# sail-sg/finetune-fair-diffusion

Measured on AMD Instinct MI355X. Metric: training-images/sec (SD-v1.5 512^2, 20-step DPM-Solver++ unroll, fairness-finetune step), higher is better.
Workload: dtype f16

## Files before the change

finetune_fair_diffusion_amd/ops.py:

```python
import ctypes
import os
import math

import torch

from . import lib as _lib

ACT = dict(none=0, silu=1, quick_gelu=2, gelu=3, relu=4, hardswish=5, hardsigmoid=6, geglu=7)
CONV_NORMAL, CONV_STRIDE2, CONV_UP2, CONV_TRANS2 = 0, 1, 2, 3
F16, F32 = _lib.torch_working_dtype(), torch.float32


def _stream():
    return ctypes.c_void_p(torch.cuda.current_stream().cuda_stream)


def _p(t):
    if t is None:
        return None
    assert t.is_cuda, "fairdiff ops need device tensors (no CPU path)"
    return ctypes.c_void_p(t.data_ptr())


DELAY = None


def _call(name, *args):
    if DELAY is not None and DELAY[2].random() < DELAY[0]:
        torch.cuda._sleep(int(DELAY[2].random() * DELAY[1]))
    L = _lib.get()
    rc = getattr(L, name)(*args)
    if rc != 0:
        raise RuntimeError(f"{name} failed ({rc}): {L.fd_last_error().decode()}")


_gemm_ws = {}


def gemm_workspace():
    dev = torch.cuda.current_device()
    key = (dev, torch.cuda.current_stream().cuda_stream)
    t = _gemm_ws.get(key)
    if t is None:
        t = torch.empty(16 << 20, dtype=F32, device=torch.device("cuda", dev))
        _gemm_ws[key] = t
    return t


class OpTimer:

    def __init__(self):
        self.shapes = []
        self.records = []

    def summary(self):
        torch.cuda.synchronize()
        agg = {}
        for variant, flops, nbytes, a, b, split in self.records:
            ms = a.elapsed_time(b)
            e = agg.setdefault(variant, [0, 0.0, 0.0, 0.0, 0])
            e[0] += 1; e[1] += flops; e[2] += ms; e[3] += nbytes; e[4] += int(split)
        self.by_shape = {}
        for (variant, flops, nbytes, a, b, split), shp in zip(self.records, self.shapes):
            e = self.by_shape.setdefault((variant,) + shp, [0, 0.0, 0.0])
            e[0] += 1; e[1] += flops; e[2] += a.elapsed_time(b)
        return {k: dict(launches=v[0], flops=v[1], ms=v[2], bytes=v[3], splitk_launches=v[4]) for k, v in agg.items()}

    def shape_table(self):
        rows = [k + (v[0], v[2], 1e3 * v[2] / v[0], v[1] / (v[2] * 1e-3) / 1e12) for k, v in self.by_shape.items()]
        return sorted(rows, key=lambda r: -r[10])


TIMER = None


GN_STATS = os.environ.get("FD_NO_GN_STATS") is None

def _gemm_call(d, conv, out=None, gn_stats=False):
    ws = gemm_workspace()
    d.workspace, d.workspace_bytes = ws.data_ptr(), ws.numel() * 4
    if gn_stats and GN_STATS:
        rows = _lib.get().fd_gemm_stats_rows(ctypes.byref(d))
        if rows > 0:
            nph = 4 if (conv and d.conv_mode == CONV_UP2PI) else 1
            st = torch.empty((nph * ((d.M + rows - 1) // rows), d.N // 10, 2), dtype=F32, device=out.device)
            d.gn_stats = st.data_ptr()
            out.gn_stats = (st, rows)
    if TIMER is None:
        _call("fd_gemm", ctypes.byref(d), _stream())
        return
    buf = ctypes.create_string_buffer(128)
    split = _lib.get().fd_gemm_kernel_name(ctypes.byref(d), buf, 128)
    a, b = torch.cuda.Event(enable_timing=True), torch.cuda.Event(enable_timing=True)
    a.record()
    _call("fd_gemm", ctypes.byref(d), _stream())
    b.record()
    nph = 4 if (conv and d.conv_mode in (4, 6)) else 1
    flops = 2.0 * nph * d.M * d.N * (d.K + d.K2) * max(d.batch, 1)
    a_elems = (d.Bn * d.H * d.W * d.Cin) if conv else d.M * d.K
    nbytes = 2.0 * max(d.batch, 1) * (a_elems + d.M * d.K2 + nph * d.N * (d.K + d.K2) + nph * d.M * d.N)
    TIMER.records.append((buf.value.decode(), flops, nbytes, a, b, split > 1))
    TIMER.shapes.append((d.M, d.N, d.K, d.K2, d.conv_mode if conv else -1, int(d.act), int(bool(d.residual)), split))


def _chk(t, dtype=F16):
    assert t.dtype == dtype and t.is_contiguous(), (t.dtype, t.shape, t.stride())
    return t


def gemm(a, b, *, a2=None, b2=None, bias=None, rowbias=None, rows_per_batch=0, residual=None, act="none", alpha=1.0,
         out=None, out_dtype=F16, n=None, aux=None, gn_stats=False, ln=None, colscale=None):
    M, K = a.shape
    N = b.shape[0] if n is None else n
    assert b.shape[1] == K and a.stride(1) == 1 and b.stride(1) == 1
    if out is None:
        out = torch.empty((M, N // 2 if act == "geglu" else N), dtype=out_dtype, device=a.device)
    d = _lib.GemmDesc()
    d.A, d.lda, d.B, d.ldb = a.data_ptr(), a.stride(0), b.data_ptr(), b.stride(0)
    if a2 is not None:
        assert a2.shape[0] == M and a2.shape[1] == b2.shape[1] and a2.stride(1) == 1 and b2.stride(1) == 1
        d.A2, d.lda2, d.B2, d.ldb2, d.K2 = a2.data_ptr(), a2.stride(0), b2.data_ptr(), b2.stride(0), a2.shape[1]
    d.C, d.ldc = out.data_ptr(), out.stride(0)
    if bias is not None:
        d.bias = _chk(bias, F32).data_ptr()
    if rowbias is not None:
        d.rowbias, d.ld_rowbias, d.rows_per_batch = _chk(rowbias).data_ptr(), rowbias.stride(0), rows_per_batch
    if residual is not None:
        assert residual.dtype == F16 and residual.stride(1) == 1
        d.residual, d.ldr = residual.data_ptr(), residual.stride(0)
    if aux is not None:
        assert act == "geglu" and residual is None and aux.shape == (M, N) and aux.dtype == F16 and aux.is_contiguous()
        d.residual, d.ldr = aux.data_ptr(), N
    d.alpha, d.M, d.N, d.K = alpha, M, N, K
    d.act, d.out_dtype, d.batch = ACT[act], 1 if out.dtype == F32 else 0, 1
    if colscale is not None:
        d.colscale, d.colscale_cols = colscale
    if ln is None:
        _gemm_call(d, False, out, gn_stats)
        return out
    _gemm_call(d, False, out, False)
    y, st = layernorm(out, ln[0], ln[1], ln[2], save_stats=True)
    return out, y, st


def interleave_geglu(w, bias):
    F = w.shape[0] // 2
    wi = torch.stack([w[:F], w[F:]], dim=1).reshape(2 * F, w.shape[1]).contiguous()
    bi = torch.stack([bias[:F], bias[F:]], dim=1).reshape(2 * F).contiguous() if bias is not None else None
    return wi, bi


def bgemm(a, b, *, alpha=1.0, out=None):
    Z, M, K = a.shape
    N = b.shape[1]
    _chk(a), _chk(b)
    if out is None:
        out = torch.empty((Z, M, N), dtype=F16, device=a.device)
    d = _lib.GemmDesc()
    d.A, d.lda, d.B, d.ldb, d.C, d.ldc = a.data_ptr(), K, b.data_ptr(), K, out.data_ptr(), N
    d.alpha, d.M, d.N, d.K, d.batch = alpha, M, N, K, Z
    d.sA, d.sB, d.sC = M * K, N * K, M * N
    _gemm_call(d, False)
    return out


def gemm_batched_into(a, b, out_view, bias, residual, Z, rows):
    K, N = a.shape[1], b.shape[0]
    assert a.shape[0] == Z * rows and out_view.shape == (Z, rows, N) and out_view.stride(2) == 1 and a.is_contiguous()
    d = _lib.GemmDesc()
    d.A, d.lda, d.B, d.ldb = a.data_ptr(), K, b.data_ptr(), b.stride(0)
    d.C, d.ldc = out_view.data_ptr(), out_view.stride(1)
    if bias is not None:
        d.bias = _chk(bias, F32).data_ptr()
    if residual is not None:
        d.residual, d.ldr, d.sR = _chk(residual).data_ptr(), residual.stride(0), 0
    d.alpha, d.M, d.N, d.K, d.batch = 1.0, rows, N, K, Z
    d.sA, d.sB, d.sC = rows * K, 0, out_view.stride(0)
    _gemm_call(d, False)
    return out_view


def gemm_batched_from(a_view, b, Z, rows):
    K, N = a_view.shape[2], b.shape[0]
    assert a_view.shape[:2] == (Z, rows) and a_view.stride(2) == 1 and b.shape[1] == K
    out = torch.empty((Z * rows, N), dtype=F16, device=b.device)
    d = _lib.GemmDesc()
    d.A, d.lda, d.B, d.ldb = a_view.data_ptr(), a_view.stride(1), b.data_ptr(), b.stride(0)
    d.C, d.ldc = out.data_ptr(), N
    d.alpha, d.M, d.N, d.K, d.batch = 1.0, rows, N, K, Z
    d.sA, d.sB, d.sC = a_view.stride(0), 0, rows * N
    _gemm_call(d, False)
    return out


def conv3x3(x, w, B, H, W, *, mode=CONV_NORMAL, bias=None, rowbias=None, residual=None, act="none", out=None, gn_stats=False):
    Cin = x.shape[1]
    Cout = w.shape[0]
    assert w.shape[1] == 9 * Cin and x.shape[0] == B * H * W
    _chk(x), _chk(w)
    if mode == CONV_NORMAL:
        Ho, Wo = H, W
    elif mode == CONV_STRIDE2:
        Ho, Wo = (H + 1) // 2, (W + 1) // 2
    else:
        Ho, Wo = 2 * H, 2 * W
    M = B * Ho * Wo
    if out is None:
        out = torch.empty((M, Cout), dtype=F16, device=x.device)
    d = _lib.GemmDesc()
    d.A, d.lda, d.B, d.ldb, d.C, d.ldc = x.data_ptr(), Cin, w.data_ptr(), 9 * Cin, out.data_ptr(), out.stride(0)
    if bias is not None:
        d.bias = _chk(bias, F32).data_ptr()
    if rowbias is not None:
        d.rowbias, d.ld_rowbias, d.rows_per_batch = _chk(rowbias).data_ptr(), rowbias.stride(0), (M if rowbias.shape[0] == 1 else Ho * Wo)
    if residual is not None:
        d.residual, d.ldr = _chk(residual).data_ptr(), residual.stride(0)
    d.alpha, d.M, d.N, d.K, d.act, d.batch = 1.0, M, Cout, 9 * Cin, ACT[act], 1
    d.out_dtype = 1 if out.dtype == F32 else 0
    d.conv, d.conv_mode, d.Bn, d.H, d.W, d.Cin, d.Ho, d.Wo = 1, mode, B, H, W, Cin, Ho, Wo
    _gemm_call(d, True, out, gn_stats)
    return out, Ho, Wo


CONV_UP2P, CONV_UP2P_BWD, CONV_UP2PI = 4, 5, 6
_BIG_TILES = (256320, 128320, 128160, 256128, 256256, 512128)
_NO_UP2P = os.environ.get("FD_NO_UP2P") is not None


def _up2p_desc(x, w, out, B, H, W, Cin, Cout, bwd, bias=None):
    d = _lib.GemmDesc()
    if bwd:
        d.K, d.conv_mode, d.H, d.W = 16 * Cin, CONV_UP2P_BWD, 2 * H, 2 * W
    else:
        d.K, d.conv_mode, d.H, d.W = 4 * Cin, CONV_UP2PI, H, W
    d.A, d.lda, d.B, d.ldb, d.C, d.ldc = x.data_ptr(), Cin, w.data_ptr(), d.K, out.data_ptr(), Cout
    if bias is not None:
        d.bias = _chk(bias, F32).data_ptr()
    d.alpha, d.M, d.N, d.act, d.batch, d.out_dtype = 1.0, B * H * W, Cout, ACT["none"], 1, 0
    d.conv, d.Bn, d.Cin, d.Ho, d.Wo = 1, B, Cin, H, W
    ws = gemm_workspace()
    d.workspace, d.workspace_bytes = ws.data_ptr(), ws.numel() * 4
    return d


def conv_up2(x, conv, B, H, W):
    Cin, Cout = conv.cin, conv.cout
    if not _NO_UP2P and Cin % 64 == 0 and Cout % 8 == 0:
        out = torch.empty((4 * B * H * W, Cout), dtype=F16, device=x.device)
        d = _up2p_desc(_chk(x), conv.wk_up2p, out, B, H, W, Cin, Cout, False, conv.bias)
        if _lib.get().fd_gemm_tile(ctypes.byref(d)) in _BIG_TILES:
            _gemm_call(d, True, out, gn_stats=(H * W) % 32 == 0)
            if getattr(out, "gn_stats", None) is not None:
                out.gn_stats = out.gn_stats + ((H * W) // 32,)
            return out, 2 * H, 2 * W
    return conv3x3(x, conv.wk, B, H, W, mode=CONV_UP2, bias=conv.bias)


def conv_up2_bwd(dy, conv, B, H, W):
    Cin, Cout = conv.cin, conv.cout
    if not _NO_UP2P and Cout % 64 == 0 and Cin % 8 == 0:
        out = torch.empty((B * H * W, Cin), dtype=F16, device=dy.device)
        d = _up2p_desc(_chk(dy), conv.wd_up2p, out, B, H, W, Cout, Cin, True)
        if _lib.get().fd_gemm_tile(ctypes.byref(d)) % 1000000 in _BIG_TILES:
            _gemm_call(d, True)
            return out
    dxu, _, _ = conv3x3(dy, conv.wd, B, 2 * H, 2 * W)
    return downsum2x2(dxu, B, H, W, Cin)


def conv_small_cin(x, w, bias, B, H, W, Cin, Cout, k, stride=1, nchw=True, act="none"):
    pad = (k - 1) // 2
    Ho, Wo = (H + 2 * pad - k) // stride + 1, (W + 2 * pad - k) // stride + 1
    y = torch.empty((B * Ho * Wo, Cout), dtype=F16, device=x.device)
    assert x.is_contiguous() and x.dtype in (F16, F32)
    _call("fd_conv_small_cin", _p(x), int(x.dtype == F32), int(nchw), _p(_chk(w, F32)), _p(bias), _p(y), B, H, W, Cin, Cout, k, stride,
          ACT[act], _stream())
    return y, Ho, Wo


def conv_small_cin_bwd(dy, w, B, H, W, Cin, Cout, k, stride=1, scale=1.0):
    dx = torch.empty((B, Cin, H, W), dtype=F32, device=dy.device)
    _call("fd_conv_small_cin_bwd", _p(_chk(dy)), _p(_chk(w, F32)), _p(dx), B, H, W, Cin, Cout, k, stride, scale, _stream())
    return dx


def nhwc_to_nchw(x, B, HW, C, *, out_dtype=F32, scale=1.0, lo=-math.inf, hi=math.inf):
    y = torch.empty((B, C, HW), dtype=out_dtype, device=x.device)
    _call("fd_nhwc_to_nchw", _p(x), x.stride(0), _p(y), int(out_dtype == F32), B, HW, C, scale, lo, hi, _stream())
    return y


def clamp_bwd(pre, dimg, B, HW, C, lo=-1.0, hi=1.0):
    out = torch.empty_like(dimg)
    _call("fd_clamp_bwd", _p(pre), pre.stride(0), _p(_chk(dimg, F32)), _p(out), B, HW, C, lo, hi, _stream())
    return out
# ... 432 lines not shown
```

finetune_fair_diffusion_amd/unet.py:

```python
import math

import torch

from . import ops
from .layers import (F16, F32, Conv3x3, Linear, LoRAPair, Norm, ParamBank, ResnetBlock, lora_linear_bwd, lora_linear_fwd)
from .weights import UNetConfig, unet_attn_names, unet_lora_param_shapes, unet_param_shapes


BWD_SLOT = [None]


class _Out:
    def __init__(self, sample):
        self.sample = sample


class LoRAAttnProcessor:

    def __init__(self, hidden_size, cross_attention_dim=None, rank=4):
        self.hidden_size, self.cross_attention_dim, self.rank = hidden_size, cross_attention_dim, rank

    def to(self, *a, **k):
        return self


class AttnLoRA:

    def __init__(self, bank, name):
        self.q, self.k, self.v, self.out = (LoRAPair(bank, f"{name}.{p}_lora.down.weight", f"{name}.{p}_lora.up.weight")
                                            for p in ("to_q", "to_k", "to_v", "to_out"))
        dev = bank.flat.device
        rp = self.q.rp
        if self.q.K == self.k.K:
            C = self.q.N
            self.down_qkv16 = torch.zeros((3 * rp, C), dtype=F16, device=dev)
            self.down_qkvT16 = torch.zeros((C, 3 * rp), dtype=F16, device=dev)
            self.up_qkv16 = torch.zeros((3 * C, 3 * rp), dtype=F16, device=dev)
            self.upT_qkv16 = torch.zeros((3 * rp, 3 * C), dtype=F16, device=dev)
            for i, p in enumerate((self.q, self.k, self.v)):
                p.place(self.down_qkv16[i * rp:(i + 1) * rp], self.down_qkvT16[:, i * rp:(i + 1) * rp],
                        self.up_qkv16[i * C:(i + 1) * C, i * rp:(i + 1) * rp], self.upT_qkv16[i * rp:(i + 1) * rp, i * C:(i + 1) * C])
            self.down_kv16 = self.down_qkv16[rp:]
        else:
            self.down_kv16 = torch.zeros((2 * rp, self.k.K), dtype=F16, device=dev)
            self.q.place()
            self.k.place(down16=self.down_kv16[:rp])
            self.v.place(down16=self.down_kv16[rp:])
        self.out.place()

    def pairs(self):
        return (self.q, self.k, self.v, self.out)

    def refresh(self):
        from .layers import refresh_pairs
        refresh_pairs(self.pairs())


class TransformerBlock:

    def __init__(self, sd, p, dev, C, heads, groups, xdim):
        self.C, self.heads, self.d, self.groups, self.xdim = C, heads, C // heads, groups, xdim
        self.p = p
        self.norm = Norm(sd, p + "norm", dev)
        self.proj_in = Linear(sd, p + "proj_in", dev, conv1x1=True)
        self.proj_out = Linear(sd, p + "proj_out", dev, conv1x1=True)
        b = p + "transformer_blocks.0."
        self.ln1, self.ln2, self.ln3 = Norm(sd, b + "norm1", dev), Norm(sd, b + "norm2", dev), Norm(sd, b + "norm3", dev)
        self.q1, self.k1, self.v1, self.o1 = (Linear(sd, b + "attn1." + n, dev) for n in ("to_q", "to_k", "to_v", "to_out.0"))
        assert self.q1.bias is None and self.k1.bias is None and self.v1.bias is None
        self.wqkv = torch.cat([self.q1.w, self.k1.w, self.v1.w], 0).contiguous()
        self._wqkvT = None
        self.q2, self.k2, self.v2, self.o2 = (Linear(sd, b + "attn2." + n, dev) for n in ("to_q", "to_k", "to_v", "to_out.0"))
        ff1, self.ff2 = Linear(sd, b + "ff.net.0.proj", dev), Linear(sd, b + "ff.net.2", dev)
        self.ff1_wi, self.ff1_bi = ops.interleave_geglu(ff1.w, ff1.bias)
        self._ff1_wiT = None
        self.lora1 = self.lora2 = None
        self.name1, self.name2 = b + "attn1.processor", b + "attn2.processor"
        self.cross = None
        self.lean = False

    def prepare_cross(self, enc, Bk, L, record, static=False):
        lo = self.lora2
        te = ops.gemm(enc, lo.down_kv16) if lo is not None else None
        rp = lo.k.rp if lo is not None else 0
        old = None
        if lo is not None:
            K = ops.gemm(enc, self.k2.w, a2=te[:, :rp], b2=lo.k.up16)
            V = ops.gemm(enc, self.v2.w, a2=te[:, rp:], b2=lo.v.up16)
        elif static:
            old = self.cross if (self.cross is not None and self.cross.get("static") and self.cross["K"].shape == (Bk * L, self.C)) else None
            K = ops.gemm(enc, self.k2.w, out=old["K"] if old else None)
            V = ops.gemm(enc, self.v2.w, out=old["V"] if old else None)
            if old is None:
                self.static_generation = getattr(self, "static_generation", 0) + 1
        else:
            K, V = ops.gemm(enc, self.k2.w), ops.gemm(enc, self.v2.w)
        self.cross = dict(static=bool(static and lo is None), K=K, V=V, Bk=Bk, L=L, enc=enc, te=te)
        if ops.FUSED_CROSS and L <= ops.CROSS_LP and self.C in ops.CROSS_WIDTHS and self.heads == 8:
            self.cross["Vt80"] = ops.transpose_btc(V, Bk, L, self.C, ops.CROSS_LP, out=old.get("Vt80") if (static and old) else None)
        if record:
            self.cross["dK"] = torch.zeros((Bk * L, self.C), dtype=F32, device=enc.device)
            self.cross["dV"] = torch.zeros((Bk * L, self.C), dtype=F32, device=enc.device)

    def finish_cross_backward(self, gscale, need_denc):
        c, lo = self.cross, self.lora2
        if c.get("slots") is not None:
            c["dK"] += c["slots"][:, 0].sum(dim=0)
            c["dV"] += c["slots"][:, 1].sum(dim=0)
            c["slots"] = None
        dK, dV = ops.to_f16(c["dK"]), ops.to_f16(c["dV"])
        rp = lo.k.rp if lo is not None else 0
        te = c["te"]
        denc = lora_linear_bwd(dK, c["enc"], te[:, :rp] if te is not None else None, self.k2, lo.k if lo else None, gscale, need_dx=need_denc)
        denc = lora_linear_bwd(dV, c["enc"], te[:, rp:] if te is not None else None, self.v2, lo.v if lo else None, gscale, residual=denc,
                               need_dx=need_denc)
        return denc

    def forward(self, x, B, H, W, ctx=None, pair=False):
        HW, C, h, d = H * W, self.C, self.heads, self.d
        rec = ctx is not None
        g, st = ops.groupnorm(x, None, B, HW, self.groups, 1e-6, self.norm.gamma, self.norm.beta, False)
        h0, n1, ln1 = ops.gemm(g, self.proj_in.w, bias=self.proj_in.bias, ln=(self.ln1.gamma, self.ln1.beta, 1e-5))
        l1 = self.lora1
        qs = ops.q_prescale(d)
        csq = (qs, C) if qs is not None else None
        if l1 is not None:
            t1 = ops.gemm(n1, l1.down_qkv16)
            qkv = ops.gemm(n1, self.wqkv, a2=t1, b2=l1.up_qkv16, colscale=csq)
        else:
            t1 = None
            qkv = ops.gemm(n1, self.wqkv, colscale=csq)
        q, k, v = qkv[:, :C], qkv[:, C:2 * C], qkv[:, 2 * C:]
        o, lse = ops.attn_fwd(q, k, v, B, h, HW, HW, d, 1, need_lse=True, prescaled=qs is not None)
        l2 = self.lora2
        cr = self.cross
        if (not pair and cr.get("Vt80") is not None and self.q2.bias is None and self.o2.bias is not None and (ops.FUSED_CROSS_TRAIN or (not rec and l2 is None))
                and ops.cross_block_ok(B * HW, C, h, cr["L"], HW, l2.q.rp if l2 is not None else 0)):
            h1, to1 = lora_linear_fwd(o, self.o1, l1.out if l1 else None, residual=h0)
            qs2 = ops.q_prescale(d)
            h2, n3, ln3, r = ops.cross_attn_block(h1, (self.ln2.gamma, self.ln2.beta, 1e-5), self.q2.w, cr["K"], cr["Vt80"], cr["L"], self.o2.w, self.o2.bias,
                                                  (self.ln3.gamma, self.ln3.beta, 1e-5), h, HW, B // cr["Bk"], lora_q=l2.q if l2 else None,
                                                  lora_o=l2.out if l2 else None, record=rec, q_prescaled=qs2 is not None)
            lean = rec and self.lean
            proj = torch.empty((n3.shape[0], self.ff1_wi.shape[0]), dtype=F16, device=n3.device) if rec and not lean else None
            gg = ops.gemm(n3, self.ff1_wi, bias=self.ff1_bi, act="geglu", aux=proj)
            h3 = ops.gemm(gg, self.ff2.w, bias=self.ff2.bias, residual=h2)
            out = ops.gemm(h3, self.proj_out.w, bias=self.proj_out.bias, residual=x, gn_stats=True)
            if rec:
                ctx.append(dict(x=x, st=st, h0=h0, ln1=ln1, n1=None if lean else n1, t1=t1, qkv=qkv, o=o, lse=lse, to1=to1, h1=h1, ln2=r["ln2"], n2=None if lean else r["n2"], tq2=r["tq2"], q2=r["q2"],
                                o2=r["o2"], lse2=r["lse2"], to2=r["to2"], h2=h2, ln3=ln3, proj=proj, pair=False, qs=qs is not None, qs2=qs2 is not None))
            return out
        (h1, n2, ln2), to1 = lora_linear_fwd(o, self.o1, l1.out if l1 else None, residual=h0, ln=(self.ln2.gamma, self.ln2.beta, 1e-5))
        qs2 = ops.q_prescale(d)
        q2, tq2 = lora_linear_fwd(n2, self.q2, l2.q if l2 else None, colscale=(qs2, C) if qs2 is not None else None)
        B2 = 2 * B if pair else B
        q2f, h1f, xf = (torch.cat([q2, q2]), torch.cat([h1, h1]), torch.cat([x, x])) if pair else (q2, h1, x)
        kv_div = B2 // cr["Bk"]
        o2, lse2 = ops.attn_fwd(q2f, cr["K"], cr["V"], B2, h, HW, cr["L"], d, kv_div, need_lse=True, prescaled=qs2 is not None)
        (h2, n3, ln3), to2 = lora_linear_fwd(o2, self.o2, l2.out if l2 else None, residual=h1f, ln=(self.ln3.gamma, self.ln3.beta, 1e-5))
        lean = rec and self.lean
        proj = torch.empty((n3.shape[0], self.ff1_wi.shape[0]), dtype=F16, device=n3.device) if rec and not lean else None
        gg = ops.gemm(n3, self.ff1_wi, bias=self.ff1_bi, act="geglu", aux=proj)
        h3 = ops.gemm(gg, self.ff2.w, bias=self.ff2.bias, residual=h2)
        out = ops.gemm(h3, self.proj_out.w, bias=self.proj_out.bias, residual=xf, gn_stats=True)
        if rec:
            ctx.append(dict(x=x, st=st, h0=h0, ln1=ln1, n1=None if lean else n1, t1=t1, qkv=qkv, o=o, lse=lse, to1=to1, h1=h1, ln2=ln2, n2=None if lean else n2,
                            tq2=tq2, q2=q2f, o2=o2, lse2=lse2, to2=to2, h2=h2, ln3=ln3, proj=proj, pair=pair, qs=qs is not None, qs2=qs2 is not None))
        return out

    def backward(self, d_out, B, H, W, c, gscale, need_dx=True):
        with ops.wgrad_batch():
            return self._backward(d_out, B, H, W, c, gscale, need_dx)

    def _backward(self, d_out, B, H, W, c, gscale, need_dx=True):
        HW, C, h, d = H * W, self.C, self.heads, self.d
        l1, l2 = self.lora1, self.lora2
        pair = c.get("pair", False)
        dh3 = ops.gemm(d_out, self.proj_out.wT)
        dgg = ops.gemm(dh3, self.ff2.wT)
        proj = c["proj"]
        if proj is None:
            proj = ops.gemm(ops.layernorm(c["h2"], self.ln3.gamma, self.ln3.beta, 1e-5), self.ff1_wi, bias=self.ff1_bi)
        dproj = ops.geglu_bwd_interleaved(proj, dgg)
        del proj
        if self._ff1_wiT is None:
            self._ff1_wiT = self.ff1_wi.t().contiguous()
        dn3 = ops.gemm(dproj, self._ff1_wiT)
        dh2 = ops.layernorm_bwd(c["h2"], dn3, self.ln3.gamma, c["ln3"], add=dh3)
        do2 = lora_linear_bwd(dh2, c["o2"], c["to2"], self.o2, l2.out if l2 else None, gscale)
        cr = self.cross
        kv_div = B // cr["Bk"]
        slot = BWD_SLOT[0] if cr.get("slots") is not None else None
        if slot is not None:
            dq2, _, _ = ops.attn_bwd(c["q2"], cr["K"], cr["V"], c["o2"], do2, c["lse2"], B, h, HW, cr["L"], d, kv_div,
                                     dk_out=cr["slots"][slot, 0], dv_out=cr["slots"][slot, 1], prescaled=c.get("qs2", False))
        else:
            dq2, _, _ = ops.attn_bwd(c["q2"], cr["K"], cr["V"], c["o2"], do2, c["lse2"], B, h, HW, cr["L"], d, kv_div,
                                     dk_acc=cr["dK"], dv_acc=cr["dV"], prescaled=c.get("qs2", False))
        if pair:
            B = B // 2
            M = B * HW
            dq2 = ops.add(dq2[:M], dq2[M:])
            dh2 = ops.add(dh2[:M], dh2[M:])
            if need_dx:
                d_out = ops.add(d_out[:M], d_out[M:])
        n2 = c["n2"] if (c["n2"] is not None or l2 is None) else ops.layernorm(c["h1"], self.ln2.gamma, self.ln2.beta, 1e-5)
        dn2 = lora_linear_bwd(dq2, n2, c["tq2"], self.q2, l2.q if l2 else None, gscale)
        dh1 = ops.layernorm_bwd(c["h1"], dn2, self.ln2.gamma, c["ln2"], add=dh2)
        do1 = lora_linear_bwd(dh1, c["o"], c["to1"], self.o1, l1.out if l1 else None, gscale)
        qkv = c["qkv"]
        dqkv = torch.empty_like(qkv)
        ops.attn_bwd(qkv[:, :C], qkv[:, C:2 * C], qkv[:, 2 * C:], c["o"], do1, c["lse"], B, h, HW, HW, d, 1, dqkv=dqkv, prescaled=c.get("qs", False))
        if self._wqkvT is None:
            self._wqkvT = self.wqkv.t().contiguous()
        if l1 is not None:
            t1, rp = c["t1"], l1.q.rp
            n1 = c["n1"] if c["n1"] is not None else ops.layernorm(c["h0"], self.ln1.gamma, self.ln1.beta, 1e-5)
            u = ops.gemm(dqkv, l1.upT_qkv16)
            for i, pair in enumerate((l1.q, l1.k, l1.v)):
                gd, gu = pair.grads()
                ops.lora_wgrad(dqkv[:, i * C:(i + 1) * C], t1[:, i * rp:(i + 1) * rp], gu, pair.r, 1, pair.r, scale=1.0 / gscale)
                ops.lora_wgrad(n1, u[:, i * rp:(i + 1) * rp], gd, 1, pair.K, pair.r, scale=1.0 / gscale)
            dn1 = ops.gemm(dqkv, self._wqkvT, a2=u, b2=l1.down_qkvT16) if need_dx else None
        else:
            dn1 = ops.gemm(dqkv, self._wqkvT) if need_dx else None
        if not need_dx:
            return None
        dh0 = ops.layernorm_bwd(c["h0"], dn1, self.ln1.gamma, c["ln1"], add=dh1)
        dg = ops.gemm(dh0, self.proj_in.wT)
        dx, _ = ops.groupnorm_bwd(c["x"], None, dg, B, HW, self.groups, c["st"], self.norm.gamma, self.norm.beta, False, add1=d_out)
        return dx


class UNet2DConditionModel:
    def __init__(self, cfg: UNetConfig, state_dict, device):
        self.config, self.device = cfg, device
        shapes = unet_param_shapes(cfg)
        missing = [k for k in shapes if k not in state_dict]
        if missing:
            raise KeyError(f"UNet state_dict is missing {len(missing)} tensors, e.g. {missing[:3]}")
        sd, dev = state_dict, device
        boc, g, heads, xdim, n = cfg.block_out_channels, cfg.norm_num_groups, cfg.attention_head_dim, cfg.cross_attention_dim, cfg.layers_per_block
        self.temb_dim = boc[0] * 4
        w = sd["conv_in.weight"].to(dev, F32)
        self.conv_in_w = w.permute(2, 3, 1, 0).reshape(9 * cfg.in_channels, boc[0]).contiguous()
        self.conv_in_b = sd["conv_in.bias"].to(dev, F32).contiguous()
        self.time1, self.time2 = Linear(sd, "time_embedding.linear_1", dev), Linear(sd, "time_embedding.linear_2", dev)
        self.resnets, self.transformers = [], []

        def res(p):
            r = ResnetBlock(sd, p, dev, g, 1e-5)
            self.resnets.append(r)
            return r

        def tr(p, c):
            t = TransformerBlock(sd, p, dev, c, heads, g, xdim)
            self.transformers.append(t)
            return t

        self.down = []
        cout = boc[0]
        for i, t in enumerate(cfg.down_block_types):
            cout = boc[i]
            blk = dict(res=[res(f"down_blocks.{i}.resnets.{j}.") for j in range(n)],
                       attn=[tr(f"down_blocks.{i}.attentions.{j}.", cout) for j in range(n)] if t.startswith("CrossAttn") else None,
                       down=Conv3x3(sd, f"down_blocks.{i}.downsamplers.0.conv", dev) if i != len(boc) - 1 else None)
            self.down.append(blk)
        c = boc[-1]
        self.mid = dict(res=[res("mid_block.resnets.0."), res("mid_block.resnets.1.")], attn=[tr("mid_block.attentions.0.", c)])
        self.up = []
        rev = list(reversed(boc))
        for i, t in enumerate(cfg.up_block_types):
            cout = rev[i]
            blk = dict(res=[res(f"up_blocks.{i}.resnets.{j}.") for j in range(n + 1)],
                       attn=[tr(f"up_blocks.{i}.attentions.{j}.", cout) for j in range(n + 1)] if t.startswith("CrossAttn") else None,
                       up=Conv3x3(sd, f"up_blocks.{i}.upsamplers.0.conv", dev) if i != len(boc) - 1 else None)
            self.up.append(blk)
        self.norm_out = Norm(sd, "conv_norm_out", dev)
        self.conv_out = Conv3x3(sd, "conv_out", dev)
        wo = sd["conv_out.weight"].to(dev, F32)
        self.conv_out_wd = wo.flip(2, 3).permute(2, 3, 0, 1).reshape(9 * cfg.out_channels, boc[0]).contiguous()
        ws, bs, off = [], [], 0
        for r in self.resnets:
            ws.append(r.temb_w.to(dev, F16))
            bs.append(r.temb_b.to(dev, F32))
            r.temb_slice = (off, off + ws[-1].shape[0])
            off += ws[-1].shape[0]
        self.temb_proj_w = torch.cat(ws, 0).contiguous()
        self.temb_proj_b = torch.cat(bs, 0).contiguous()
        self.lora_bank = None
        self._tr_by_name = {}
        for t in self.transformers:
            self._tr_by_name[t.name1] = (t, 1)
            self._tr_by_name[t.name2] = (t, 2)
        self.temb_table = None
        self._ctx = None

    @property
    def attn_processors(self):
        return {n: (getattr(self._tr_by_name[n][0], f"lora{self._tr_by_name[n][1]}")) for n in unet_attn_names(self.config)}

    def set_attn_processor(self, processors):
        names = unet_attn_names(self.config)
        if set(processors) != set(names):
            raise ValueError(f"expected {len(names)} attention processors, got {len(processors)} with different names")
        ranks = {p.rank for p in processors.values()}
        if len(ranks) != 1:
            raise ValueError(f"all LoRA processors must share one rank, got {sorted(ranks)}")
        shapes = unet_lora_param_shapes(self.config, ranks.pop())
        for n, p in processors.items():
            cin = shapes[n + ".to_k_lora.down.weight"][1]
            hid = shapes[n + ".to_q_lora.down.weight"][1]
            if p.hidden_size != hid or (p.cross_attention_dim or hid) != cin:
                raise ValueError(f"{n}: processor sizes ({p.hidden_size}, {p.cross_attention_dim}) do not match the U-Net ({hid}, {cin})")
        return self.add_lora(next(iter(processors.values())).rank, seed=getattr(next(iter(processors.values())), "seed", 0))

# ... 236 lines not shown
```

include/fairdiff_hip.h:

```cpp
#ifndef FAIRDIFF_HIP_H
#define FAIRDIFF_HIP_H
#include <stdint.h>
#ifdef __cplusplus
extern "C" {
#endif

#define FD_OK 0
#define FD_ERR_ARG (-1)
#define FD_ERR_LAUNCH (-2)
#define FD_ABI_VERSION 4

enum { FD_ACT_NONE = 0, FD_ACT_SILU = 1, FD_ACT_QUICK_GELU = 2, FD_ACT_GELU = 3, FD_ACT_RELU = 4,
       FD_ACT_HARDSWISH = 5, FD_ACT_HARDSIGMOID = 6,
       FD_ACT_GEGLU = 7 };
enum { FD_OUT_F16 = 0, FD_OUT_F32 = 1 };
enum { FD_CONV_NORMAL = 0, FD_CONV_STRIDE2 = 1, FD_CONV_UP2 = 2, FD_CONV_TRANS2 = 3,
       FD_CONV_UP2P = 4,
       FD_CONV_UP2P_BWD = 5,
       FD_CONV_UP2PI = 6 };

const char* fd_last_error(void);
int fd_version(void);
const char* fd_working_dtype(void);
const char* fd_build_info(void);

typedef struct fd_gemm_desc {
    int32_t struct_size;
    const void* A;  int64_t lda;
    const void* B;  int64_t ldb;
    const void* A2; int64_t lda2;
    const void* B2; int64_t ldb2;
    void* C;        int64_t ldc;
    const float* bias;
    const void* rowbias; int64_t ld_rowbias; int32_t rows_per_batch;
    const void* residual; int64_t ldr;
    float alpha;
    int32_t M, N, K, K2;
    int32_t act, out_dtype;
    int32_t batch; int64_t sA, sB, sC, sR;
    int32_t conv, conv_mode, Bn, H, W, Cin, Ho, Wo;
    void* workspace; int64_t workspace_bytes;
    float* gn_stats;
    float colscale; int32_t colscale_cols;
} fd_gemm_desc;
int fd_gemm(const fd_gemm_desc* d, void* stream);
int fd_gemm_stats_rows(const fd_gemm_desc* d);
int fd_gemm_tile(const fd_gemm_desc* d);
int fd_gemm_kernel_name(const fd_gemm_desc* d, char* buf, int n);

int fd_conv_small_cin(const void* x, int x_is_f32, int nchw, const float* w, const float* bias, void* y,
                      int B, int H, int W, int Cin, int Cout, int ksize, int stride, int act, void* stream);
int fd_nhwc_to_nchw(const void* x, int64_t ldx, void* y, int y_is_f32, int B, int HW, int C, float scale, float lo, float hi, void* stream);
int fd_clamp_bwd(const void* pre, int64_t ldx, const float* dimg, float* dpre, int B, int HW, int C, float lo, float hi, void* stream);

int fd_groupnorm_fwd(const void* x1, int C1, const void* x2, int C2, int B, int HW, int groups, float eps, const float* gamma,
                     const float* beta, int silu, void* y, float* mean_rstd, float* scratch, void* stream);
int fd_groupnorm_fwd_stats(const void* x1, int C1, const void* x2, int C2, int B, int HW, int groups, float eps, const float* gamma,
                           const float* beta, int silu, void* y, float* mean_rstd, const float* st1, int rows1, const float* st2, int rows2,
                           void* stream);
int fd_groupnorm_fwd_stats_p(const void* x1, int C1, const void* x2, int C2, int B, int HW, int groups, float eps, const float* gamma,
                             const float* beta, int silu, void* y, float* mean_rstd, const float* st1, int rows1, int per1, const float* st2,
                             int rows2, int per2, void* stream);
int fd_groupnorm_bwd(const void* x1, int C1, const void* x2, int C2, const void* dy, int B, int HW, int groups,
                     const float* mean_rstd, const float* gamma, const float* beta, int silu,
                     float* scratch, const void* add1, const void* add2, void* dx1, void* dx2, void* stream);

int fd_layernorm_fwd(const void* x, const float* gamma, const float* beta, void* y, float* mean_rstd ,
                     int M, int C, float eps, void* stream);
int fd_layernorm_bwd(const void* x, const void* dy, const float* gamma, const float* mean_rstd, const void* add ,
                     void* dx, int M, int C, void* stream);

int fd_geglu_fwd(const void* proj , void* y , int M, int F, void* stream);
int fd_geglu_bwd(const void* proj, const void* dy, void* dproj, int M, int F, void* stream);
int fd_geglu_bwd_interleaved(const void* proj, const void* dy, void* dproj, int M, int F, void* stream);
int fd_act_fwd(const void* x, void* y, int64_t n, int act, void* stream);
int fd_act_bwd(const void* z, const void* dy, void* dx, int64_t n, int act, void* stream);
int fd_add(const void* a, const void* b, void* y, int64_t n, float sa, float sb, void* stream);
int fd_copy_cols(const void* src, int64_t lds, void* dst, int64_t ldd, int64_t M, int cols, void* stream);
int fd_transpose_btc(const void* x , int64_t ldx, void* y , int B, int T, int C, int Tp, void* stream);
int fd_downsum2x2(const void* x , void* y , int B, int H, int W, int C, void* stream);
int fd_softmax_rows(const void* x, void* y, int64_t rows, int cols, float scale, const float* mask, int mask_t, int mask_ht, void* stream);
int fd_softmax_rows_bwd(const void* p, const void* dp, void* ds, int64_t rows, int cols, float scale, void* stream);
int fd_cast_f32_to_f16(const float* x, void* y, int64_t n, float scale, void* stream);
int fd_cast_f16_to_f32(const void* x, float* y, int64_t n, float scale, void* stream);

int fd_attn_fwd(const void* q, const void* k, const void* v, void* o, float* lse, int B, int H, int Tq, int Tk,
                int Tkr, int d, int kv_div, float scale, int ldq, int ldk, void* stream);
int fd_attn_bwd_prep(const void* o, const void* d_o, float* D, int B, int H, int T, int d, void* stream);
int fd_attn_bwd_dq(const void* q, const void* k, const void* v, const void* d_o, const float* lse,
                   float* D, const void* o, void* dq, int B, int H, int Tq, int Tk, int Tkr, int d, int kv_div, float scale,
                   int ldq, int ldkv, int lddq, void* stream);
int fd_attn_bwd_dkdv(const void* q, const void* k, const void* v, const void* d_o,
                     const float* lse, const float* D, void* dk, void* dv, int B, int H, int Tq, int Tk, int Tkr, int d,
                     int kv_div, float scale, int ldq, int ldkv, int lddkv, int accumulate, void* stream);
int fd_sum_slabs(const float* in, float* out, int nslab, int64_t n, void* stream);

typedef struct fd_cross_block_desc {
    int32_t struct_size;
    const void* x;
    const float* ln2_gamma; const float* ln2_beta; float ln2_eps;
    const void* wq;
    const void* k; const void* vt; int32_t L, Lp;
    const void* wo; const float* bo;
    const float* ln3_gamma; const float* ln3_beta; float ln3_eps;
    void* y; void* yn; float* yn_stats;
    int32_t M, C, heads, rows_per_sample, kv_div;
    float scale;
    const void* lora_q_down; int64_t ld_q_down; const void* lora_q_up; int64_t ld_q_up;
    const void* lora_o_down; int64_t ld_o_down; const void* lora_o_up; int64_t ld_o_up;
    int32_t lora_rp;
    void* n2_out; float* ln2_stats; void* q_out; void* tq_out; void* o_out; float* lse_out; void* to_out;
    int32_t q_prescaled;
} fd_cross_block_desc;
int fd_cross_attn_block(const fd_cross_block_desc* d, void* stream);

int fd_small_attn_fwd(const void* q, const void* k, const void* v, void* o, float* P, const int32_t* key_valid, int B, int H, int T,
                      int d, float scale, int causal, void* stream);
int fd_small_attn_bwd(const void* q, const void* k, const void* v, const float* P, const void* d_o, void* dq, void* dk, void* dv,
                      int B, int H, int T, int d, float scale, void* stream);

int fd_lora_wgrad(const void* X, int64_t ldx, const void* T, int64_t ldt, float* G, int64_t g_stride_n, int64_t g_stride_r,
                  int M, int N, int R, float scale, float* scratch, int64_t scratch_elems, void* stream);

#define FD_WGRAD_MAX 16
typedef struct fd_wgrad_desc {
    int32_t struct_size;
    const void* X; int64_t ldx;
    const void* T; int64_t ldt;
    float* G; int64_t g_stride_n, g_stride_r;
    int32_t M, N, R;
    float scale;
} fd_wgrad_desc;
int fd_lora_wgrad_multi(const fd_wgrad_desc* descs, int n, float* scratch, int64_t scratch_elems, void* stream);

typedef struct fd_lora_refresh_desc {
    int32_t struct_size;
    const float* down; const float* up;
    void* d16; int64_t ld_d16;
    void* dT16; int64_t ld_dT16;
    void* u16; int64_t ld_u16;
    void* uT16; int64_t ld_uT16;
    int32_t r, rp, K, N;
    float scale;
} fd_lora_refresh_desc;
int fd_lora_refresh_multi(const fd_lora_refresh_desc* descs, int n, void* stream);

int fd_cfg_dpm_step(const float* eps, float guidance, float* lat, const float* x0_prev, float* x0_out,
                    float alpha_t, float sigma_t, float c_x, float c_d0, float c_d1, int64_t n, void* stream);

int fd_grad_finite_scale(float* g, int64_t n, float scale, int32_t* nonfinite_flag, void* stream);
int fd_adamw_ema(float* p, const float* g, float* m, float* v, float* ema, int64_t n, float lr, float beta1, float beta2,
                 float eps, float weight_decay, int32_t step, float ema_one_minus_decay, void* stream);

int fd_dwconv_fwd(const void* x, const float* w , const float* bias, void* y, int B, int H, int W, int C,
                  int k, int stride, int act, void* stream);
int fd_dwconv_bwd(const void* dy, const float* w, void* dx, int B, int H, int W, int C, int k, int stride, void* stream);
int fd_avgpool_hw(const void* x, void* y, int B, int HW, int C, void* stream);
int fd_avgpool_hw_bwd(const void* dy , const void* add , void* dx, int B, int HW, int C, void* stream);
int fd_scale_channels(const void* x, const void* s, void* y, int B, int HW, int C, void* stream);
int fd_scale_channels_bwd(const void* x, const void* s, const void* dy, void* dx, void* ds , int B, int HW, int C, void* stream);
int fd_conv_small_cin_bwd(const void* dy , const float* w, float* dx ,
                          int B, int H, int W, int Cin, int Cout, int ksize, int stride, float scale, void* stream);
int fd_crop_resize_fwd(const void* img, const int32_t* boxes, float fill, void* chips, int B, int H, int W, int S, void* stream);
int fd_crop_resize_bwd(const float* dchips , const int32_t* boxes, float* dimg ,
                       int B, int H, int W, int S, void* stream);

int fd_patchify_fwd(const void* chips, void* patches, const float* mean3, const float* std3, int N, int S, int P, int Kp, void* stream);
int fd_patchify_bwd(const void* dpatches, float* dchips, const float* std3, int N, int S, int P, int Kp, float scale, int accumulate,
                    void* stream);
int fd_warp_affine_fwd(const void* img, const int32_t* src_index, const float* A, float fill, void* chips, int n_chips, int H, int W,
                       int S, void* stream);
int fd_warp_affine_bwd(const float* dchips, const int32_t* src_index, const float* A, float* dimg, int n_chips, int B, int H, int W,
                       int S, void* stream);
int fd_rect_scale(float* dimg, const int32_t* rects, const float* factors, int B, int H, int W, void* stream);

int fd_ot_assign_sum(const double* cost, const int32_t* counts, float* plan, int32_t* seats, int N, int K, int S, void* stream);
int fd_ot_expected_targets(const double* cost, const int32_t* counts, const double* weights, int32_t* seats, int32_t* targets, double* uncertainty,
                           int N, int K, int S, void* stream);

#ifdef __cplusplus
}
#endif
#endif
```

Baseline: 6.313.

## Fuse transformer feed-forward GEGLU GEMM and down-projection into one kernel for C=320

Adds a HIP kernel that computes the FF1 GEMM with bias and erf-GELU gating, keeps the gated activations in LDS, and runs the FF2 GEMM with bias and residual epilogue in the same block. Weight tiles stream through a prefetched LDS ring. The goal is to skip the round trip of the 4C-wide GEGLU intermediate through global memory and to save one launch per transformer block at the C=320 level. Other widths fall back to the two-GEMM path. The tradeoff is that each block recomputes over the full weights, so the weights get reread per 128-row tile, and the fixed LDS-heavy schedule may limit occupancy.

New measurement: 6.273, median of 2. About the same (-0.6%).

```diff
diff --git a/finetune_fair_diffusion_amd/csrc/ffblock.hip b/finetune_fair_diffusion_amd/csrc/ffblock.hip
--- /dev/null
+++ b/finetune_fair_diffusion_amd/csrc/ffblock.hip
@@ -0,0 +1,196 @@
+#include "gemm_pp_device.h"
+
+namespace {
+constexpr int FFB_C = 320, FFB_BM = 128, FFB_NW = 8;
+constexpr int FFB_F2 = 8 * FFB_C;
+constexpr int FFB_K2 = 4 * FFB_C;
+constexpr int FFB_NCH = FFB_K2 / 64;
+constexpr int FFB_KS1 = FFB_C / 32;
+constexpr int FFB_STEPS = FFB_KS1 + 2 * (FFB_C / 16) / FFB_NW;
+constexpr int FFB_SLOTS = 7, FFB_PF = 4;
+static_assert(FFB_PF <= FFB_SLOTS - 3, "ring: the W2 groups of a step are read up to two steps later");
+constexpr int FFB_GG = FFB_KS1 * 8;
+constexpr int FFB_RING = FFB_GG + 16;
+constexpr size_t FFB_LDS = (size_t)(FFB_RING + FFB_SLOTS * 8) * PP_GROUP * sizeof(f16);
+constexpr uint32_t FFB_OOR = 0xFFFFFFF0u;
+typedef uint32_t v2u32 __attribute__((ext_vector_type(2)));
+
+struct FfbArgs {
+    const f16 *x, *w1, *w2;
+    const float* b1;
+    f16* proj;
+    int M;
+};
+}
+
+template <bool PROJ>
+__global__ __launch_bounds__(512) void ff_block_kernel(FfbArgs a, fd_gemm_desc ep) {
+    extern __shared__ __attribute__((aligned(16))) f16 smem[];
+    const int tid = threadIdx.x, lane = tid & 63;
+    const int wave = __builtin_amdgcn_readfirstlane(tid >> 6);
+    const int l15 = lane & 15, lg = lane >> 4;
+    const int wm = wave >> 2, wn = wave & 3;
+    const int m0 = blockIdx.x * FFB_BM;
+    const int M = a.M;
+
+    const int lrow = lane >> 2;
+    const int kchunk = ((lane & 3) ^ swz_g(lane >> 4)) * 8;
+#if __HIP_DEVICE_COMPILE__
+    auto rsrc = [](const void* base, int64_t bytes) { return __builtin_amdgcn_make_buffer_rsrc((void*)base, 0, (int)(uint32_t)bytes, 0x00020000); };
+    const __amdgpu_buffer_rsrc_t rX = rsrc(a.x, (int64_t)M * FFB_C * 2), rW1 = rsrc(a.w1, (int64_t)FFB_F2 * FFB_C * 2),
+                                 rW2 = rsrc(a.w2, (int64_t)FFB_C * FFB_K2 * 2), rB1 = rsrc(a.b1, (int64_t)FFB_F2 * 4),
+                                 rP = rsrc(a.proj, PROJ ? (int64_t)M * FFB_F2 * 2 : 0);
+    const int xrow = m0 + wave * 16 + lrow;
+    const uint32_t x_vo = xrow < M ? (uint32_t)(xrow * FFB_C + kchunk) * 2 : FFB_OOR;
+    auto lds_at = [&](int group) { return (__attribute__((address_space(3))) void*)(smem + group * PP_GROUP); };
+
+    auto issue = [&](int T) {
+        const int slot = T % FFB_SLOTS;
+        auto dst = lds_at(FFB_RING + slot * 8 + wave);
+        if (T >= FFB_NCH * FFB_STEPS) {
+            __builtin_amdgcn_raw_ptr_buffer_load_lds(rW1, dst, 16, FFB_OOR, 0, 0, 0);
+            return;
+        }
+        const int c = T / FFB_STEPS, st = T - c * FFB_STEPS;
+        if (st < FFB_KS1) {
+            const uint32_t vo = (uint32_t)((c * 128 + wave * 16 + lrow) * FFB_C + kchunk) * 2;
+            __builtin_amdgcn_raw_ptr_buffer_load_lds(rW1, dst, 16, vo, (uint32_t)st * 64, 0, 0);
+        } else {
+            const int g = (st - FFB_KS1) * 8 + wave;
+            const int h = g >= 20 ? 1 : 0;
+            const uint32_t vo = (uint32_t)(((g - 20 * h) * 16 + lrow) * FFB_K2 + kchunk) * 2;
+            __builtin_amdgcn_raw_ptr_buffer_load_lds(rW2, dst, 16, vo, (uint32_t)(c * 64 + h * 32) * 2, 0, 0);
+        }
+    };
+
+#pragma unroll
+    for (int s = 0; s < FFB_KS1; ++s) __builtin_amdgcn_raw_ptr_buffer_load_lds(rX, lds_at(s * 8 + wave), 16, x_vo, (uint32_t)s * 64, 0, 0);
+#pragma unroll
+    for (int T = 0; T < FFB_PF; ++T) issue(T);
+
+    f32x4 acc[4][5];
+#pragma unroll
+    for (int i = 0; i < 4; ++i)
+#pragma unroll
+        for (int j = 0; j < 5; ++j) acc[i][j] = (f32x4){0.f, 0.f, 0.f, 0.f};
+
+    const uint32_t lds0 = (uint32_t)(uintptr_t)(__attribute__((address_space(3))) void*)smem;
+    const uint32_t frag = (uint32_t)(l15 * 32 + ((lg ^ swz_g(l15 >> 2)) * 8)) * 2;
+    constexpr uint32_t GB = PP_GROUP * 2;
+    const uint32_t gg_wr = lds0 + (uint32_t)(FFB_GG + (wn >> 1) * 8 + wm * 4) * GB + (uint32_t)(l15 * 32 + lg * 2) * 2;
+    const int prow = m0 + wm * 64 + l15;
+    auto nop = [] {};
+
+#pragma unroll 1
+    for (int c = 0; c < FFB_NCH; ++c) {
+        f32x4 acc1[4][2];
+        f32x4 bias1[2];
+        static_for<0, FFB_STEPS>([&](auto stc) {
+            constexpr int st = decltype(stc)::value;
+            const int T = c * FFB_STEPS + st;
+            constexpr int XB = (st >= 1 && st <= 3) ? 2 : 0;
+            constexpr int XP = (PROJ && st >= 10 && st <= 13) ? 8 : 0;
+            wait_vm<FFB_PF - 1 + XB + XP>();
+            raw_barrier();
+            issue(T + FFB_PF);
+            const uint32_t slot_b = lds0 + (uint32_t)(FFB_RING + (T % FFB_SLOTS) * 8) * GB;
+            if constexpr (st == 0) {
+#pragma unroll
+                for (int i = 0; i < 4; ++i) acc1[i][0] = acc1[i][1] = (f32x4){0.f, 0.f, 0.f, 0.f};
+#pragma unroll
+                for (int j = 0; j < 2; ++j)
+                    bias1[j] = __builtin_bit_cast(f32x4, __builtin_amdgcn_raw_buffer_load_b128(rB1, (uint32_t)(c * 128 + wn * 32 + j * 16 + lg * 4) * 4, 0, 0));
+            }
+            if constexpr (st < FFB_KS1) {
+                mma_k32_mid<4, 2, 2, GB, false, decltype(nop)&>(acc1, lds0 + (uint32_t)(st * 8 + wm * 4) * GB + frag, slot_b + (uint32_t)(wn * 2) * GB + frag, nop);
+            }
+            if constexpr (st == FFB_KS1 - 1) {
+#pragma unroll
+                for (int i = 0; i < 4; ++i) {
+#pragma unroll
+                    for (int j = 0; j < 2; ++j) {
+                        const f32x4 v = acc1[i][j] + bias1[j];
+                        const f16 v0 = (f16)v[0], g0 = (f16)v[1], v1 = (f16)v[2], g1 = (f16)v[3];
+                        const f16x2 o = {(f16)((float)v0 * gelu_erf_f((float)g0)), (f16)((float)v1 * gelu_erf_f((float)g1))};
+                        const uint32_t slot = (uint32_t)((((wn & 1) * 2 + j) ^ swz_g(l15 >> 2)) * 16);
+                        asm volatile("ds_write_b32 %0, %1" ::"v"(gg_wr + (uint32_t)i * GB + slot), "v"(__builtin_bit_cast(uint32_t, o)) : "memory");
+                        if constexpr (PROJ) {
+                            const int m = prow + i * 16;
+                            const uint32_t off = m < M ? (uint32_t)(m * FFB_F2 + c * 128 + wn * 32 + j * 16 + lg * 4) * 2 : FFB_OOR;
+                            const f16x4 pv = {v0, g0, v1, g1};
+                            __builtin_amdgcn_raw_buffer_store_b64(__builtin_bit_cast(v2u32, pv), rP, off, 0, 0);
+                        }
+                    }
+                }
+                asm volatile("s_waitcnt lgkmcnt(0)" ::: "memory");
+            }
+            if constexpr (st == FFB_KS1 + 2 || st == FFB_STEPS - 1) {
+                constexpr int h = st == FFB_STEPS - 1 ? 1 : 0;
+                const int T0 = c * FFB_STEPS + FFB_KS1;
+                f16x8 af[4], bf[5];
+                const uint32_t a_addr = lds0 + (uint32_t)(FFB_GG + h * 8 + wm * 4) * GB + frag;
+                static_for<0, 4>([&](auto ic) {
+                    constexpr int i = decltype(ic)::value;
+                    ds_read16<i * GB>(af[i], a_addr);
+                });
+                static_for<0, 5>([&](auto jc) {
+                    constexpr int j = decltype(jc)::value;
+                    const int g = h * 20 + wn * 5 + j;
+                    const uint32_t addr = lds0 + (uint32_t)(FFB_RING + ((T0 + (g >> 3)) % FFB_SLOTS) * 8 + (g & 7)) * GB + frag;
+                    ds_read16<0>(bf[j], addr);
+                });
+                wait_lgkm<0>();
+#pragma unroll
+                for (int i = 0; i < 4; ++i) tie(af[i]);
+#pragma unroll
+                for (int j = 0; j < 5; ++j) tie(bf[j]);
+#pragma unroll
+                for (int i = 0; i < 4; ++i)
+#pragma unroll
+                    for (int j = 0; j < 5; ++j) acc[i][j] = FD_MFMA_16x16x32(bf[j], af[i], acc[i][j]);
+            }
+        });
+    }
+    asm volatile("s_waitcnt vmcnt(0)" ::: "memory");
+    __syncthreads();
+    gemm_epilogue_lds<4, 5, 4, false>(ep, acc, smem + wave * (64 * 84), m0 + wm * 64, wn * 80, lane, 0, 0);
+#endif
+}
+
+extern "C" int fd_ff_block_takes(int M, int C) {
+#ifdef FD_BENCH_HOOKS
+    const char* e = getenv("FD_FF_FUSED");
+    if (e && atoi(e) == 0) return 0;
+#endif
+    return C == FFB_C && M > 0 && (int64_t)M * FFB_F2 < (1LL << 30) ? 1 : 0;
+}
+
+extern "C" int fd_ff_block(const void* x, const void* w1, const float* b1, const void* w2, const float* b2, const void* residual, void* out, void* proj,
+                           int M, int C, void* stream) {
+    FD_REQUIRE(fd_ff_block_takes(M, C), "fd_ff_block: M = %d, C = %d not supported (C = 320, M * 8C < 2^30)", M, C);
+    FD_REQUIRE(x && w1 && b1 && w2 && b2 && residual && out, "fd_ff_block: NULL operand");
+    fd_gemm_desc ep{};
+    ep.struct_size = sizeof(fd_gemm_desc);
+    ep.C = out;
+    ep.ldc = FFB_C;
+    ep.bias = b2;
+    ep.residual = residual;
+    ep.ldr = FFB_C;
+    ep.alpha = 1.f;
+    ep.M = M;
+    ep.N = FFB_C;
+    ep.K = FFB_K2;
+    ep.batch = 1;
+    ep.act = FD_ACT_NONE;
+    ep.out_dtype = FD_OUT_F16;
+    FfbArgs a{(const f16*)x, (const f16*)w1, (const f16*)w2, b1, (f16*)proj, M};
+    const dim3 grid((M + FFB_BM - 1) / FFB_BM);
+    static std::once_flag once;
+    std::call_once(once, [] {
+        (void)hipFuncSetAttribute((const void*)ff_block_kernel<false>, hipFuncAttributeMaxDynamicSharedMemorySize, (int)FFB_LDS);
+        (void)hipFuncSetAttribute((const void*)ff_block_kernel<true>, hipFuncAttributeMaxDynamicSharedMemorySize, (int)FFB_LDS);
+    });
+    if (proj) hipLaunchKernelGGL(ff_block_kernel<true>, grid, dim3(512), FFB_LDS, (hipStream_t)stream, a, ep);
+    else hipLaunchKernelGGL(ff_block_kernel<false>, grid, dim3(512), FFB_LDS, (hipStream_t)stream, a, ep);
+    return fd_check_launch("fd_ff_block");
+}
diff --git a/finetune_fair_diffusion_amd/ops.py b/finetune_fair_diffusion_amd/ops.py
--- a/finetune_fair_diffusion_amd/ops.py
+++ b/finetune_fair_diffusion_amd/ops.py
@@ -141,6 +141,22 @@
     _gemm_call(d, False, out, False)
     y, st = layernorm(out, ln[0], ln[1], ln[2], save_stats=True)
     return out, y, st
+
+
+def ff_block_takes(M, C):
+    return bool(_lib.get().fd_ff_block_takes(M, C))
+
+
+def ff_block(x, w1i, b1i, w2, b2, residual, proj=None):
+    M, C = x.shape
+    if not (ff_block_takes(M, C) and b1i is not None and b2 is not None and x.is_contiguous() and residual.is_contiguous()):
+        return gemm(gemm(x, w1i, bias=b1i, act="geglu", aux=proj), w2, bias=b2, residual=residual)
+    assert w1i.shape == (8 * C, C) and w2.shape == (C, 4 * C) and residual.shape == (M, C)
+    assert proj is None or (proj.shape == (M, 8 * C) and proj.dtype == F16 and proj.is_contiguous())
+    out = torch.empty_like(x)
+    _call("fd_ff_block", _p(_chk(x)), _p(_chk(w1i)), _p(_chk(b1i, F32)), _p(_chk(w2)), _p(_chk(b2, F32)), _p(_chk(residual)), _p(out), _p(proj),
+          M, C, _stream())
+    return out
 
 
 def interleave_geglu(w, bias):
diff --git a/finetune_fair_diffusion_amd/unet.py b/finetune_fair_diffusion_amd/unet.py
--- a/finetune_fair_diffusion_amd/unet.py
+++ b/finetune_fair_diffusion_amd/unet.py
@@ -143,8 +143,7 @@
                                                   lora_o=l2.out if l2 else None, record=rec, q_prescaled=qs2 is not None)
             lean = rec and self.lean
             proj = torch.empty((n3.shape[0], self.ff1_wi.shape[0]), dtype=F16, device=n3.device) if rec and not lean else None
-            gg = ops.gemm(n3, self.ff1_wi, bias=self.ff1_bi, act="geglu", aux=proj)
-            h3 = ops.gemm(gg, self.ff2.w, bias=self.ff2.bias, residual=h2)
+            h3 = ops.ff_block(n3, self.ff1_wi, self.ff1_bi, self.ff2.w, self.ff2.bias, h2, proj=proj)
             out = ops.gemm(h3, self.proj_out.w, bias=self.proj_out.bias, residual=x, gn_stats=True)
             if rec:
                 ctx.append(dict(x=x, st=st, h0=h0, ln1=ln1, n1=None if lean else n1, t1=t1, qkv=qkv, o=o, lse=lse, to1=to1, h1=h1, ln2=r["ln2"], n2=None if lean else r["n2"], tq2=r["tq2"], q2=r["q2"],
@@ -160,8 +159,7 @@
         (h2, n3, ln3), to2 = lora_linear_fwd(o2, self.o2, l2.out if l2 else None, residual=h1f, ln=(self.ln3.gamma, self.ln3.beta, 1e-5))
         lean = rec and self.lean
         proj = torch.empty((n3.shape[0], self.ff1_wi.shape[0]), dtype=F16, device=n3.device) if rec and not lean else None
-        gg = ops.gemm(n3, self.ff1_wi, bias=self.ff1_bi, act="geglu", aux=proj)
-        h3 = ops.gemm(gg, self.ff2.w, bias=self.ff2.bias, residual=h2)
+        h3 = ops.ff_block(n3, self.ff1_wi, self.ff1_bi, self.ff2.w, self.ff2.bias, h2, proj=proj)
         out = ops.gemm(h3, self.proj_out.w, bias=self.proj_out.bias, residual=xf, gn_stats=True)
         if rec:
             ctx.append(dict(x=x, st=st, h0=h0, ln1=ln1, n1=None if lean else n1, t1=t1, qkv=qkv, o=o, lse=lse, to1=to1, h1=h1, ln2=ln2, n2=None if lean else n2,
diff --git a/include/fairdiff_hip.h b/include/fairdiff_hip.h
--- a/include/fairdiff_hip.h
+++ b/include/fairdiff_hip.h
@@ -64,6 +64,10 @@
 int fd_groupnorm_bwd(const void* x1, int C1, const void* x2, int C2, const void* dy, int B, int HW, int groups,
                      const float* mean_rstd, const float* gamma, const float* beta, int silu,
                      float* scratch, const void* add1, const void* add2, void* dx1, void* dx2, void* stream);
+
+int fd_ff_block_takes(int M, int C);
+int fd_ff_block(const void* x, const void* w1, const float* b1, const void* w2, const float* b2, const void* residual, void* out, void* proj,
+                int M, int C, void* stream);
 
 int fd_layernorm_fwd(const void* x, const float* gamma, const float* beta, void* y, float* mean_rstd ,
                      int M, int C, float eps, void* stream);
```
